# jibanCat/gp_dla_detection

Measured on AMD Instinct MI355X. Metric: sample log-likelihoods/sec (n~1500,k=20), higher is better.
Workload: dtype f64; 1 GPU; BASELINE configs[1]: synthetic spectra, fused Voigt + low-rank log-evidence sweep, HBM-resident; spectra_per_gpu=1000, pixels=1500, k=20, dla_samples=10000, num_lines=3, parallelism=spectra sharded over 1 GPU(s), RCCL all-gather of the 15-column posterior table

## Files before the change

gp_dla_detection_amd/csrc/sweep_kernels.hpp:

```cpp
#pragma once
#include <hip/hip_runtime.h>
#include <stdint.h>

#include <type_traits>
#include <utility>

#include "faddeeva.hpp"
#include "near_tables.hpp"

namespace gpdla {

typedef double d4 __attribute__((ext_vector_type(4)));

typedef float f4 __attribute__((ext_vector_type(4)));

template <typename T> struct Mat;
template <> struct Mat<double> {
  using acc_t = d4;
  static __device__ __forceinline__ acc_t mfma(double a, double b, acc_t c) {
    return __builtin_amdgcn_mfma_f64_16x16x4f64(a, b, c, 0, 0, 0);
  }
  static __device__ __forceinline__ int sample_of(int jj, int r) { return jj + 4 * r; }
  static __device__ __forceinline__ int jj_of(int sample) { return sample & 3; }
  static __device__ __forceinline__ int reg_of(int sample) { return sample >> 2; }
// ... 427 lines not shown
  p = fma(p, r, 0.16666666666666666);
  p = fma(p, r, 0.5);
  p = fma(p, r, 1.0);
  p = fma(p, r, 1.0);
  return ldexp(p, (int)n);
}

constexpr double kE1 = 0x1.7fffffffd940ep+0, kE2 = 0x1.e0000294b4cbcp+1, kE3 = 0x1.a3f92a26b3728p+3,
                 kE4 = 0x1.df9f0e43cd754p+5;
__device__ __forceinline__ double wing_lead(double rho, double e3v) {
  double t;
  asm("v_fma_f64 %0, %1, %2, %3" : "=v"(t) : "v"(rho), "s"(kE4), "v"(e3v));
  return t;
}

__device__ __forceinline__ double wing_core(double x2, double y2) {
  const double rho = fast_rcp(x2 + y2);
  double t = fma(kE4, rho, kE3);
  t = fma(t, rho, kE2);
  t = fma(t, rho, kE1);
  t = fma(t, rho, 1.0);
  t = fma(-2.0 * y2 * rho, rho, t);
  return rho * t;
}

__device__ __forceinline__ void glds16(const double *gsrc, double *lds_wave_base) {
  const uint32_t lds = __builtin_amdgcn_readfirstlane(
      (uint32_t)(uintptr_t)(__attribute__((address_space(3))) void *)lds_wave_base);
  asm volatile("s_mov_b32 m0, %1\n\ts_nop 0\n\tglobal_load_lds_dwordx4 %0, off"
               :
               : "v"(gsrc), "s"(lds)
               : "memory", "m0");
}
__device__ __forceinline__ void glds_wait() {
  __builtin_amdgcn_s_waitcnt(0x0F70);
  asm volatile("" ::: "memory");
}

constexpr int kRecordPoolPad = 8;
__device__ __forceinline__ void glds_quad(const double *gsrc, uint32_t lds, int count) {
  if (count >= 4)
    asm volatile("s_mov_b32 m0, %1\n\ts_nop 0\n\tglobal_load_lds_dwordx4 %0, off\n\t"
                 "global_load_lds_dwordx4 %0, off offset:1024\n\tglobal_load_lds_dwordx4 %0, off offset:2048\n\t"
                 "global_load_lds_dwordx4 %0, off offset:3072"
                 :
                 : "v"(gsrc), "s"(lds)
                 : "memory", "m0");
  else if (count == 3)
    asm volatile("s_mov_b32 m0, %1\n\ts_nop 0\n\tglobal_load_lds_dwordx4 %0, off\n\t"
                 "global_load_lds_dwordx4 %0, off offset:1024\n\tglobal_load_lds_dwordx4 %0, off offset:2048"
                 :
                 : "v"(gsrc), "s"(lds)
                 : "memory", "m0");
  else if (count == 2)
    asm volatile("s_mov_b32 m0, %1\n\ts_nop 0\n\tglobal_load_lds_dwordx4 %0, off\n\t"
                 "global_load_lds_dwordx4 %0, off offset:1024"
                 :
                 : "v"(gsrc), "s"(lds)
                 : "memory", "m0");
  else if (count == 1)
    asm volatile("s_mov_b32 m0, %1\n\ts_nop 0\n\tglobal_load_lds_dwordx4 %0, off" : : "v"(gsrc), "s"(lds) : "memory", "m0");
}
template <int KIB, int WAVES>
__device__ __forceinline__ void glds_chunk(const double *src, uint32_t lds, int wave, int lane) {
  constexpr int PER = (KIB + WAVES - 1) / WAVES;
  const int first = wave * PER;
// ... 414 lines not shown
  return q_s + ld_s + e[0];
#else
  if (role != 0) return NAN;
  if (TW <= 14)
    return factor_rows<ES::ROWS, ES::LPS, 20>(e + half * ncols, s & (ES::LPS - 1), k, voff, q_s, ld_s, n_kept);
#ifndef GPDLA_EXP_LDSEPI
  if constexpr (TW > 30 && ES::LPS == 16) {
    Rows16<40> R;
    load_rows16<40>(R, e, s, k, voff);
    return factor_rows16<40>(R, k, q_s, ld_s, n_kept);
  }
#endif
  return factor_lds<ES::ROWS, ES::LPS>(e + half * ncols, s & (ES::LPS - 1), k, voff, q_s, ld_s, n_kept);
#endif
}

__device__ __forceinline__ double near_poly(const double *line_tab, double ax) {
  const bool core = ax < 8.0;
  const double u = core ? ax * 8.0 : (ax - 8.0) * 2.0;
  const int i = (int)u;
  const double t = (u - (double)i) - 0.5;
  const double *c = line_tab + (size_t)((core ? 0 : kNearCore) + i) * kNearCoef;
  double cf[kNearCoef];
#pragma unroll
  for (int k = 0; k < kNearCoef; ++k) cf[k] = c[k];
  double p = cf[kNearCoef - 1];
#pragma unroll
  for (int k = kNearCoef - 2; k >= 0; --k) p = fma(p, t, cf[k]);
  return p;
}

__device__ __forceinline__ uint32_t hi_word(double v) { return (uint32_t)__double2hiint(v); }

__device__ __forceinline__ double wing_sum3(double lamP, double msa, double msb, double msc, double cs,
                                            bool *near) {
  const double xa = fma(lamP, msa, -cs), xb = fma(lamP, msb, -cs), xc = fma(lamP, msc, -cs);
  const double sa = fma(xa, xa, g_lines.y2[0]), sb = fma(xb, xb, g_lines.y2[1]), sc = fma(xc, xc, g_lines.y2[2]);
  static_assert(__builtin_bit_cast(unsigned long long, 900.0) == 0x408C200000000000ull, "bits of 900.0");
  *near = min(min(hi_word(sa), hi_word(sb)), hi_word(sc)) < 0x408C2000u;
  const double pab = sa * sb, pbc = sb * sc, pac = sa * sc;
  const double rinv = fast_rcp(pab * sc);
  const double ra = rinv * pbc, rb = rinv * pac, rc = rinv * pab;
  double ta = ra * kE4 + kE3, tb = rb * kE4 + kE3, tc = rc * kE4 + kE3;
  ta = fma(ta, ra, g_lines.t2[0]); tb = fma(tb, rb, g_lines.t2[1]); tc = fma(tc, rc, g_lines.t2[2]);
  ta = fma(ta, ra, kE1); tb = fma(tb, rb, kE1); tc = fma(tc, rc, kE1);
  ta = fma(ta, ra, 1.0); tb = fma(tb, rb, 1.0); tc = fma(tc, rc, 1.0);
  return fma(g_lines.cwing[2], rc * tc, fma(g_lines.cwing[1], rb * tb, g_lines.cwing[0] * (ra * ta)));
}

__device__ __forceinline__ double wing_sum3_rcp4(double lamP, double msa, double msb, double msc, double cs,
                                                 bool *near, double d, double *inv_d) {
  const double xa = fma(lamP, msa, -cs), xb = fma(lamP, msb, -cs), xc = fma(lamP, msc, -cs);
  const double sa = fma(xa, xa, g_lines.y2[0]), sb = fma(xb, xb, g_lines.y2[1]), sc = fma(xc, xc, g_lines.y2[2]);
  *near = min(min(hi_word(sa), hi_word(sb)), hi_word(sc)) < 0x408C2000u;
  const double pab = sa * sb, pabc = pab * sc;
  const double rinv = fast_rcp(pabc * d);
  *inv_d = rinv * pabc;
  const double r3 = rinv * d;
  const double rc = r3 * pab, r2 = r3 * sc;
  const double ra = r2 * sb, rb = r2 * sa;
  const double e3v = kE3;
  double ta = wing_lead(ra, e3v), tb = wing_lead(rb, e3v), tc = wing_lead(rc, e3v);
  ta = fma(ta, ra, g_lines.t2[0]); tb = fma(tb, rb, g_lines.t2[1]); tc = fma(tc, rc, g_lines.t2[2]);
  ta = fma(ta, ra, kE1); tb = fma(tb, rb, kE1); tc = fma(tc, rc, kE1);
  ta = fma(ta, ra, 1.0); tb = fma(tb, rb, 1.0); tc = fma(tc, rc, 1.0);
  return fma(g_lines.cwing[2], rc * tc, fma(g_lines.cwing[1], rb * tb, g_lines.cwing[0] * (ra * ta)));
}

constexpr int kRing2 = 33;
constexpr int kExpTab = 64;

struct ExpState {
  double r, tabv;
  int ni;
};
__device__ __forceinline__ ExpState exp_table_begin(double x, const double *tab) {
  ExpState e;
  const double nf = rint(x * 92.33248261689366);
  asm("v_cvt_i32_f64 %0, %1" : "=v"(e.ni) : "v"(nf));
  e.tabv = tab[e.ni & (kExpTab - 1)];
  e.r = fma(-nf, 0.010830424667801708, x);
  e.r = fma(-nf, 2.8447437476627285e-11, e.r);
  return e;
}
__device__ __forceinline__ double exp_table_end(const ExpState &e) {
  double p, c4 = 0.041666666666666664, c3 = 0.16666666666666666;
  asm("v_fma_f64 %0, %1, %2, %3" : "=v"(p) : "s"(0.008333333333333333), "v"(e.r), "v"(c4));
  asm("v_fma_f64 %0, %1, %2, %3" : "=v"(p) : "v"(p), "v"(e.r), "v"(c3));
  p = fma(p, e.r, 0.5);
  p = fma(p, e.r, 1.0);
  p = fma(p, e.r, 1.0);
  return ldexp(e.tabv * p, e.ni >> 6);
}
constexpr double kExpScale = 92.33248261689366;
__device__ __forceinline__ ExpState exp_table_begin_scaled(double t, const double *tab) {
  ExpState e;
  const double nf = rint(t);
  asm("v_cvt_i32_f64 %0, %1" : "=v"(e.ni) : "v"(nf));
  e.tabv = tab[e.ni & (kExpTab - 1)];
// ... 15 lines not shown
__device__ __forceinline__ double exp_table(double x, const double *tab) {
  return exp_table_end(exp_table_begin(x, tab));
}
__device__ __forceinline__ double exp_table_scaled(double t, const double *tab) {
  return exp_table_end_scaled(exp_table_begin_scaled(t, tab));
}

template <int LINES>
__device__ __forceinline__ double total_near(double lamP, double m0, double m1, double m2,
                                             const double *mult_lds, int L) {
  const double c_light = g_lines.c, inv_s = g_lines.inv_sqrt2_sigma;
  const double *tab = g_lines.near_poly;
  double total = 0.0;
  if (LINES > 0) {
    const double mm[3] = {m0, m1, m2};
#pragma unroll
    for (int j = 0; j < (LINES > 0 ? LINES : 1); ++j) {
      const double ax = fabs((lamP * mm[j < 3 ? j : 0] - c_light) * inv_s);
      const double f = ax < 30.0
                           ? 1.7724538509055159 * g_lines.leading[j] * near_poly(tab + j * kNearLineDoubles, ax)
                           : g_lines.cwing[j] * wing_core(ax * ax, g_lines.y2[j]);
      total += f;
    }
  } else {
    for (int j = 0; j < L; ++j) {
      const double ax = fabs((lamP * mult_lds[j] - c_light) * inv_s);
      const double f = ax < 30.0
                           ? 1.7724538509055159 * g_lines.leading[j] * near_poly(tab + j * kNearLineDoubles, ax)
                           : g_lines.cwing[j] * wing_core(ax * ax, g_lines.y2[j]);
      total += f;
    }
  }
  return total;
}

constexpr int kLineUnroll = 4;
__device__ __forceinline__ double wing_sum_runtime(double rho, double cs, int L, bool *near_out) {
  double total = 0.0;
  bool near = false;
  int j0 = 0;
  for (; j0 + kLineUnroll <= L; j0 += kLineUnroll) {
    double f[kLineUnroll];
#pragma unroll
    for (int u = 0; u < kLineUnroll; ++u) {
      const double x = fma(rho, g_lines.wing[j0 + u].kms, -cs);
      const double x2 = x * x;
      near |= x2 < 900.0;
      f[u] = wing_core(x2, g_lines.wing[j0 + u].y2);
    }
#pragma unroll
    for (int u = 0; u < kLineUnroll; ++u) total = fma(g_lines.wing[j0 + u].cwing, f[u], total);
  }
  for (; j0 < L; ++j0) {
    const double x = fma(rho, g_lines.wing[j0].kms, -cs);
    const double x2 = x * x;
    near |= x2 < 900.0;
    total = fma(g_lines.wing[j0].cwing, wing_core(x2, g_lines.wing[j0].y2), total);
  }
  *near_out = near;
  return total;
}

__device__ __forceinline__ double total_near_at(double lamP, double one_plus_z, int L) {
  const double c_light = g_lines.c, inv_s = g_lines.inv_sqrt2_sigma;
  const double *tab = g_lines.near_poly;
  double total = 0.0;
// ... 70 lines not shown
  if (tid < kExpTab) exp_tab[tid] = exp2((double)tid * (1.0 / kExpTab));
  double *my_ring = ring + (size_t)(wave * kSamplesPerWave + s) * kRing2 + jj;
  const double *lam = a.lam_pad + m.lam_off;
  const int n_pad = m.n_u + 6;
  const double nscale64 = -nhi * g_lines.inv_sqrt2pi_sigma * kInvSqrtPi * kExpScale;
  const double *rec_base = a.records + m.rec_off * (int64_t)RD;
  const int nchunks = (m.steps + kChunkSteps - 1) / kChunkSteps;

  static_assert((kChunkSteps * RD) % 128 == 0, "a chunk is a whole number of KiB");
  const int wave_s = __builtin_amdgcn_readfirstlane(wave);
  const uint32_t stage_lds = __builtin_amdgcn_readfirstlane(lds_address(stage));
  auto issue_chunk = [&](int c) {
    glds_chunk<kChunkSteps * RD / 128, WAVES>(rec_base + (size_t)c * kChunkSteps * RD,
                                              stage_lds + (uint32_t)(c & 1) * (uint32_t)(kChunkSteps * RD * 8), wave_s, lane);
  };
  issue_chunk(0);

  const double c_light = g_lines.c, inv_s = g_lines.inv_sqrt2_sigma;
  double ms_r[LINES > 0 ? LINES : 1];
#pragma unroll
  for (int j = 0; j < (LINES > 0 ? LINES : 0); ++j) ms_r[j] = mult_r[j] * inv_s;
  const double cs = c_light * inv_s;
#define GPDLA_TOTAL_ACCURATE(lamP)                                                        \
  total_near<LINES>((lamP), mult_r[0], mult_r[LINES > 1 ? 1 : 0], mult_r[LINES > 2 ? 2 : 0], \
                    my_mult, L)
#define GPDLA_RAW_ACCURATE(lamP) exp_table_scaled(nscale64 * GPDLA_TOTAL_ACCURATE(lamP), exp_tab)

  __syncthreads();
  for (int c3 = 0; c3 < 3; ++c3) {
    const double lam0 = lam[min(4 * c3 + jj, n_pad - 1)];
    double v;
    if (LINES == 3) {
      bool near0;
      v = exp_table_scaled(nscale64 * wing_sum3(lam0, ms_r[0], ms_r[LINES > 1 ? 1 : 0], ms_r[LINES > 2 ? 2 : 0],
                                                cs, &near0), exp_tab);
      if (__any(near0)) v = GPDLA_RAW_ACCURATE(lam0);
    } else {
      v = GPDLA_RAW_ACCURATE(lam0);
    }
    my_ring[4 * c3] = v;
    my_ring[4 * c3 + 16] = v;
  }

  acc_t acc[NTW];
#pragma unroll
  for (int c = 0; c < NTW; ++c) acc[c] = acc_t{0, 0, 0, 0};
  double quad_sum = 0.0, dprod = 1.0;
  double xw[kXW] = {0.0, 0.0}, xu[kXU] = {0.0, 0.0, 0.0, 0.0};
  int dexp = 0;
  const int tile0 = role * NTW;
  [[maybe_unused]] const int nw = TS == 1 ? TW : max(0, min(NTW, TW - tile0));
  const double tap0 = g_lines.taps[0], tap1 = g_lines.taps[1], tap2 = g_lines.taps[2],
               tap3 = g_lines.taps[3];

  glds_wait();
  __syncthreads();

#ifdef GPDLA_STAMP
  uint32_t st_sum[8] = {0, 0, 0, 0, 0, 0, 0, 0}, st_prev;
  {
    unsigned long long t0_;
    asm volatile("s_memtime %0\n\ts_waitcnt lgkmcnt(0)" : "=s"(t0_)::"memory");
    st_prev = (uint32_t)t0_;
  }
#endif
  for (int c0 = 0; c0 < nchunks; c0 += UN) {
#pragma unroll
  for (int hc = 0; hc < UN; ++hc) {
    const int c = c0 + hc;
// ... 1 lines not shown
    __builtin_amdgcn_s_waitcnt(0x0F70);
    GPDLA_ST(4)
    if (c + 1 < nchunks) issue_chunk(c + 1);
    GPDLA_ST(5)
    const double *buf = stage + (size_t)(UN > 1 ? hc : (c & 1)) * kChunkSteps * RD;
    double lam_next = 0.0;
#pragma unroll
    for (int tt = 0; tt < kChunkSteps; ++tt) {
      const int rn = c * kChunkSteps + tt;
      if (rn < m.steps) {
        const double *rec = buf + (size_t)tt * RD;
        const double *extra = rec + NT * TD;
        const int slot_p = kChunkSteps >= 4 ? (4 * tt) & 15 : (kChunkSteps == 2 ? 4 * (2 * hc + tt) : ((4 * rn) & 15));
        const int slot_w = (slot_p + 12) & 15;
        if (tt > 0) __builtin_amdgcn_s_waitcnt(0xC07F);
        const double *mine = extra + extras_row(NT, 1) * jj;
        const double lamP = tt == 0 ? extra[extras_lam_stride(NT) * jj + extras_lam(NT, 0)] : lam_next;
        const double *g = my_ring + slot_p;
        const double g0 = g[0], g1 = g[1], g2 = g[2], g3 = g[3], g4 = g[4], g5 = g[5], g6 = g[6];
        const double2 p01 = *reinterpret_cast<const double2 *>(mine);
        const double2 p23 = *reinterpret_cast<const double2 *>(mine + 2);
        const double py = p01.x, pmu = p01.y, pom = p23.x, pnu = p23.y;
        __builtin_amdgcn_sched_barrier(0);
        double absorb = g3 * tap3;
        absorb = fma(g0 + g6, tap0, absorb);
        absorb = fma(g1 + g5, tap1, absorb);
        absorb = fma(g2 + g4, tap2, absorb);
        if (is_null) absorb = 1.0;
        const double a2 = absorb * absorb;
        const double d = fma(pom, a2, pnu);
        double inv_d;
        double total;
        bool near;
        if (LINES == 3) {
          total = wing_sum3_rcp4(lamP, ms_r[0], ms_r[LINES > 1 ? 1 : 0], ms_r[LINES > 2 ? 2 : 0], cs, &near, d, &inv_d);
        } else {
          inv_d = fast_rcp(d);
          total = 0.0;
          near = false;
          for (int j = 0; j < L; ++j) {
            const double x = fma(lamP, my_mult[j] * inv_s, -cs);
            const double x2 = x * x;
            near |= x2 < 900.0;
            total = fma(g_lines.cwing[j], wing_core(x2, g_lines.y2[j]), total);
          }
        }
        GPDLA_ST(0)
#ifndef GPDLA_ABLATE_NOSLOW
        if (__builtin_expect(__any(near), 0)) total = GPDLA_TOTAL_ACCURATE(lamP);
#endif
        GPDLA_ST(1)
        const ExpState es = exp_table_begin_scaled(nscale64 * total, exp_tab);
        __builtin_amdgcn_sched_barrier(0);
        const T *bt = reinterpret_cast<const T *>(rec) + (size_t)tile0 * 64 + lane;
        T bop[NTW];
#ifdef GPDLA_ABLATE_NOBFRAG
#pragma unroll
        for (int cc = 0; cc < NTW; ++cc) bop[cc] = (T)(lane + cc) * (T)lamP;
        (void)bt;
#else
#pragma unroll
        for (int cc = 0; cc < NTW; ++cc) bop[cc] = bt[(size_t)cc * 64];
#endif
        __builtin_amdgcn_sched_barrier(0);
        double raw = exp_table_end_scaled(es);
#ifdef GPDLA_ABLATE_NOVOIGT
        raw = lamP * 1e-4;
#endif
        my_ring[slot_w] = raw;
        my_ring[slot_w + 16] = raw;
        const double r = fma(-absorb, pmu, py);
        const double w = a2 * inv_d;
        const double ri = r * inv_d;
        const double u = absorb * ri;
        quad_sum = fma(r, ri, quad_sum);
        dprod *= d;
        if (kChunkSteps == 1 || (tt & 1)) {
          dexp += __builtin_amdgcn_frexp_exp(dprod);
          dprod = __builtin_amdgcn_frexp_mant(dprod);
        }
        if (tt + 1 < kChunkSteps) {
          lam_next = extra[RD + extras_lam_stride(NT) * jj + extras_lam(NT, 0)];
// ... 282 lines not shown
```

gp_dla_detection_amd/csrc/sweep_slim_body.hpp:

```cpp
template <int LINES>
__global__ __launch_bounds__(kSlimWaves * 64, 2) void GPDLA_SWEEP_SLIM_KERNEL(GPDLA_SWEEP_SLIM_ARGS a) {
  static_assert(LINES == 3 || LINES == 0, "three lines at compile time, or a run-time count");
  extern __shared__ double smem[];
  constexpr int WAVES = kSlimWaves, CH = kSlimSweepCH;
  const int64_t xj = blockIdx.x >> 3;
  const int64_t pos = 8 * (xj / a.blocks_per_quasar) + (blockIdx.x & 7);
  const int bq = (int)(xj % a.blocks_per_quasar);
  if (pos >= a.nq) return;
  const int64_t q = a.order[pos];
  const QuasarMeta m = a.meta[q];
  if (m.status != 0) return;
  const int tid = threadIdx.x, wave = tid >> 6, lane = tid & 63;
  const int s = lane & 15, jj = lane >> 4;

  double *ring = smem;
  double *blocks = ring + kSlimSweepRingD;
  double *land = blocks + 2 * kSlimSweepBlock + wave * kSlimLand;
  const double *exp_pad = ring + 32;

  const int64_t slot0 = (int64_t)bq * (WAVES * kSamplesPerWave) + wave * kSamplesPerWave;
  const int64_t slot = slot0 + s;
  const bool is_sample = slot < a.S;
  const bool is_null = !is_sample;
  const int32_t sample = a.perm[is_sample ? slot : a.S - 1];
  const double z_dla = m.min_z_dla + (m.max_z_dla - m.min_z_dla) * a.offset_samples[sample];
  double nhi = a.nhi_samples[sample];
  if constexpr (std::is_same_v<GPDLA_SWEEP_SLIM_ARGS, BoxedSweepArgs> && LINES >= 0) {
    const double *box = sweep_box(a, q);
    nhi = exp10(box[2] + (box[3] - box[2]) * nhi);
  }
  [[maybe_unused]] double mult_r[3];
  [[maybe_unused]] const double opz = 1 + z_dla, inv_opz = 1.0 / opz;
  [[maybe_unused]] const int L = LINES > 0 ? LINES : a.num_lines;
  if constexpr (LINES == 3) {
#pragma unroll
    for (int j = 0; j < 3; ++j) mult_r[j] = g_lines.c / (g_lines.wavelength_cm[j] * (1 + z_dla)) / 1e8;
  }
  if (tid < kExpTab) ring[tid * kRing2 + 32] = exp2((double)tid * (1.0 / kExpTab));
  double *my_ring = ring + (size_t)(wave * kSamplesPerWave + s) * kRing2 + jj;
  const double *lam = a.lam_pad + m.lam_off;
  const int n_pad = m.n_u + 6;
  const double nscale64 = -nhi * g_lines.inv_sqrt2pi_sigma * kInvSqrtPi * kExpScale;
  const double *rec_base = a.records + m.rec_off * (int64_t)kSlimRec;
  const int nchunks = (m.steps + CH - 1) / CH;

  const int wave_s = __builtin_amdgcn_readfirstlane(wave);
  double *const raw_mine = blocks + kSlimSweepTileBuf + wave_s * kSlimRec;
  const double *const raw_src = rec_base + (size_t)wave_s * kSlimRec + 2 * lane;
  auto issue_chunk = [&](int c) {
    if (lane < kSlimRec / 2) glds16(raw_src + (size_t)c * CH * kSlimRec, raw_mine + (c & 1) * kSlimSweepBlock);
  };
  const double *land_src = rec_base + (size_t)wave_s * kSlimRec;
  const int src_rows = 4 * kSlimExtras + 16 * jj + 2 * (s & 7);
  const int src_x = kSlimExtras * (lane >> 1) + 4 + 2 * (lane & 1);
  auto issue_private = [&](int c) {
    const double *rec = land_src + (size_t)c * CH * kSlimRec;
    glds16(rec + src_rows, land);
    if (lane < 8) glds16(rec + src_x, land + 4 * 32);
  };
  const double *row = land + 32 * jj + s;
  const double *bc = land + 4 * 32 + 4 * jj;
  const double *a8 = s < 8 ? row : bc + (slim_pair_i(8, s) - 16);
  const double *b8 = s < 8 ? row + 8 : bc + (slim_pair_j(8, s) - 16);
  struct Operands {
    double mc, o[5], p8;
  };
  auto expand_load = [&](int t0, int t1, Operands &x) {
    x.mc = row[0];
#pragma unroll
    for (int t = t0; t < t1; ++t) {
      if (t == 8) {
        x.o[t - t0] = a8[0];
        x.p8 = b8[0];
      } else {
        x.o[t - t0] = t == 0 ? x.mc : t < 8 ? row[t] : bc[t - 9];
      }
    }
  };
  auto expand_store = [&](double *dst, int t0, int t1, const Operands &x) {
#pragma unroll
    for (int t = t0; t < t1; ++t) dst[t * 64] = (t == 8 ? x.p8 : x.mc) * x.o[t - t0];
  };
  double *const xd0 = blocks + (size_t)wave_s * kSlimStepTiles + lane;
  const double *const tb0 = blocks + lane;
  const double *const mb0 = blocks + kSlimSweepTileBuf + kSlimExtras * jj;
  const double *const ub0 = blocks + kSlimSweepTileBuf + 4 * kSlimExtras + lane;
  auto pinned = [](const double *p) {
    uint32_t v = lds_address(p);
    asm volatile("" : "+v"(v));
    return (double *)(__attribute__((address_space(3))) double *)(uintptr_t)v;
  };

  issue_private(0);
  issue_chunk(0);

  const double c_light = g_lines.c, inv_s = g_lines.inv_sqrt2_sigma;
  [[maybe_unused]] double ms_r[3];
  if constexpr (LINES == 3) {
#pragma unroll
    for (int j = 0; j < 3; ++j) ms_r[j] = mult_r[j] * inv_s;
  }
  const double cs = c_light * inv_s;
  auto optical_sum = [&](double lamP) -> double {
    if constexpr (LINES == 3) {
      bool near;
      double total = wing_sum3(lamP, ms_r[0], ms_r[1], ms_r[2], cs, &near);
      if (__builtin_expect(__any(near), 0)) total = total_near<3>(lamP, mult_r[0], mult_r[1], mult_r[2], nullptr, 3);
      return total;
    } else {
      bool near;
      double total = wing_sum_runtime(lamP * inv_opz, cs, L, &near);
      if (__builtin_expect(__any(near), 0)) total = total_near_at(lamP, opz, L);
      return total;
    }
  };

  __syncthreads();
  for (int c3 = 0; c3 < 3; ++c3) {
    const double lam0 = lam[min(4 * c3 + jj, n_pad - 1)];
    const double tot = optical_sum(lam0);
    const ExpState es0 = exp_ring_begin_scaled(nscale64 * tot, exp_pad);
    const double v = exp_table_end_scaled(es0);
    my_ring[4 * c3] = v;
    my_ring[4 * c3 + 16] = v;
  }

  d4 acc[14];
#pragma unroll
  for (int c = 0; c < 14; ++c) acc[c] = d4{0, 0, 0, 0};
  double quad_sum = 0.0, dprod = 1.0;
  double xw[kXW] = {0.0, 0.0}, xu[kXU] = {0.0, 0.0, 0.0, 0.0};
  int dexp = 0;
  const double tap0 = g_lines.taps[0], tap1 = g_lines.taps[1], tap2 = g_lines.taps[2], tap3 = g_lines.taps[3];

  glds_wait();
  {
    const double mc = row[0];
    for (int t = 0; t < kSlimTilesW; ++t)
      xd0[t * 64] = (t == 8 ? b8[0] : mc) * (t == 8 ? a8[0] : t == 0 ? mc : t < 8 ? row[t] : bc[t - 9]);
  }
  __builtin_amdgcn_s_waitcnt(0xC07F);
  if (nchunks > 1) issue_private(1);
  glds_wait();
  __syncthreads();

  double n0 = my_ring[0], n1 = my_ring[1], n2 = my_ring[2], n3 = my_ring[3], n4 = my_ring[4], n5 = my_ring[5], n6 = my_ring[6];
  for (int c = 0; c < nchunks; ++c) {
    __builtin_amdgcn_s_waitcnt(0x0070);
    if (c + 1 < nchunks) issue_chunk(c + 1);
    const int par = (c & 1) * kSlimSweepBlock;
    const double *tbuf = pinned(tb0 + par);
    const double *mine0 = pinned(mb0 + par);
    const double *ubuf = pinned(ub0 + par);
    double *xdst = pinned(xd0 + (kSlimSweepBlock - par));
    double lam_next = 0.0;
    double2 n01 = {0.0, 0.0}, n23 = {0.0, 0.0};
#pragma unroll
    for (int tt = 0; tt < CH; ++tt) {
      const int rn = c * CH + tt;
      constexpr int kXS = 3;
      constexpr int kT0[3] = {0, 5, 9}, kT1[3] = {5, 9, 13};
      if (tt == kXS && c + 2 < nchunks) issue_private(c + 2);
      if (rn < m.steps) {
        const double *tl = tbuf + (size_t)tt * kSlimStepTiles;
        const double *mine = mine0 + (size_t)tt * kSlimRec;
        const int slot_p = (4 * tt) & 15;
        const int slot_w = (slot_p + 12) & 15;
        if (tt > 0) __builtin_amdgcn_s_waitcnt(0xC07F);
        const double lamP = tt == 0 ? mine[10] : lam_next;
        double g0 = n0, g1 = n1, g2 = n2, g3 = n3, g4 = n4, g5 = n5, g6 = n6;
        double2 p01 = n01, p23 = n23;
        if (tt == 0) {
          p01 = *reinterpret_cast<const double2 *>(mine);
          p23 = *reinterpret_cast<const double2 *>(mine + 2);
        }
        const double py = p01.x, pmu = p01.y, pom = p23.x, pnu = p23.y;
        __builtin_amdgcn_sched_barrier(0);
        [[maybe_unused]] WingFront wf;
        [[maybe_unused]] bool near = false;
        if constexpr (LINES == 3) {
          if (tt == 0) {
            wf = wing3_front(lamP, ms_r[0], ms_r[1], ms_r[2], cs, &near);
            __builtin_amdgcn_sched_barrier(0);
          }
        }
        double absorb = g3 * tap3;
        absorb = fma(g0 + g6, tap0, absorb);
        absorb = fma(g1 + g5, tap1, absorb);
        absorb = fma(g2 + g4, tap2, absorb);
        if (is_null) absorb = 1.0;
        const double a2 = absorb * absorb;
        const double d = fma(pom, a2, pnu);
        double inv_d;
        double total;
        if constexpr (LINES == 3) {
          if (tt > 0) wf = wing3_front(lamP, ms_r[0], ms_r[1], ms_r[2], cs, &near);
          total = wing3_back_rcp4(wf, d, &inv_d);
#ifndef SLIM_EXP_NONEAR
          if (__builtin_expect(__any(near), 0)) total = total_near<3>(lamP, mult_r[0], mult_r[1], mult_r[2], nullptr, 3);
#endif
        } else {
          total = optical_sum(lamP);
          inv_d = fast_rcp(d);
        }
        const ExpState es = exp_ring_begin_scaled(nscale64 * total, exp_pad);
        __builtin_amdgcn_sched_barrier(0);
        double bop[14];
#pragma unroll
        for (int cc = 0; cc < kSlimTilesW; ++cc) bop[cc] = tl[cc * 64];
        bop[13] = ubuf[(size_t)tt * kSlimRec];
        __builtin_amdgcn_sched_barrier(0);
        const double pser = exp_series_scaled(es);
        const double r = fma(-absorb, pmu, py);
        const double w = a2 * inv_d;
        const double ri = r * inv_d;
        const double u = absorb * ri;
        quad_sum = fma(r, ri, quad_sum);
        dprod *= d;
        if (tt & 1) {
          dexp += __builtin_amdgcn_frexp_exp(dprod);
          dprod = __builtin_amdgcn_frexp_mant(dprod);
        }
        __builtin_amdgcn_sched_barrier(0);
        const double raw = exp_finish_scaled(es, pser);
        my_ring[slot_w] = raw;
        my_ring[slot_w + 16] = raw;
        Operands x;
        if (tt < kXS) expand_load(kT0[tt < kXS ? tt : 0], kT1[tt < kXS ? tt : 0], x);
        if (tt + 1 < CH) lam_next = mine[kSlimRec + 10];
        __builtin_amdgcn_sched_barrier(0);
        constexpr int kSplit = 11;
        const double2 xp = *reinterpret_cast<const double2 *>(mine + 8);
// ... 66 lines not shown
```

gp_dla_detection_amd/csrc/sweep_slim_kernel.hpp:

```cpp
#pragma once
#include <type_traits>

#include "sweep_kernels.hpp"

namespace gpdla {

constexpr int kSlimExtras = 12;
constexpr int kSlimRec = 4 * kSlimExtras + 64;
constexpr int kSlimCH = 8;
constexpr int kSlimTilesW = 13;
constexpr int kSlimStepTiles = kSlimTilesW * 64;
constexpr int kSlimTileBuf = kSlimCH * kSlimStepTiles;
constexpr int kSlimRawBuf = kSlimCH * kSlimRec;
constexpr int kSlimLand = 4 * 32 + 4 * 4;
constexpr int kSlimBlock = kSlimTileBuf + kSlimRawBuf;
static_assert((kSlimBlock * 8) % 512 == 0, "both parities reachable with ds_read2st64 offsets");
static_assert((kSlimCH * kSlimRec) % 128 == 0, "a raw chunk is a whole number of KiB");
constexpr int kSlimWaves = 4;
constexpr int kSlimSweepCH = 4;
constexpr int kSlimSweepRingD = kSlimWaves * kSamplesPerWave * kRing2;
constexpr int kSlimSweepTileBuf = kSlimSweepCH * kSlimStepTiles;
constexpr int kSlimSweepBlock = kSlimSweepTileBuf + kSlimSweepCH * kSlimRec;
constexpr int kSlimLdsDoubles = kSlimSweepRingD + 2 * kSlimSweepBlock + kSlimWaves * kSlimLand;
static_assert(kSlimSweepCH == kSlimWaves, "wave w expands, and copies, K-step w of the next chunk");
// ... 70 lines not shown
__device__ __forceinline__ ExpState exp_ring_begin_scaled(double t, const double *ring_pad) {
  ExpState e;
  const double nf = rint(t);
  asm("v_cvt_i32_f64 %0, %1" : "=v"(e.ni) : "v"(nf));
  e.tabv = ring_pad[(e.ni & (kExpTab - 1)) * kRing2];
  e.r = t - nf;
  return e;
}

__device__ __forceinline__ double exp_series_scaled(const ExpState &e) {
  constexpr double L = 0.010830424696249145;
  constexpr double c1 = L, c2 = L * L / 2, c3 = L * L * L / 6, c4 = L * L * L * L / 24, c5 = L * L * L * L * L / 120;
  double p;
  const double c4v = c4;
  asm("v_fma_f64 %0, %1, %2, %3" : "=v"(p) : "s"(c5), "v"(e.r), "v"(c4v));
  asm("v_fma_f64 %0, %1, %2, %3" : "=v"(p) : "v"(p), "v"(e.r), "s"(c3));
  asm("v_fma_f64 %0, %1, %2, %3" : "=v"(p) : "v"(p), "v"(e.r), "s"(c2));
  asm("v_fma_f64 %0, %1, %2, %3" : "=v"(p) : "v"(p), "v"(e.r), "s"(c1));
  return fma(p, e.r, 1.0);
}
__device__ __forceinline__ double exp_finish_scaled(const ExpState &e, double p) { return ldexp(e.tabv * p, e.ni >> 6); }

struct WingFront {
  double sa, sb, sc, pab, pabc;
};
__device__ __forceinline__ WingFront wing3_front(double lamP, double msa, double msb, double msc, double cs, bool *near) {
  WingFront f;
  const double xa = fma(lamP, msa, -cs), xb = fma(lamP, msb, -cs), xc = fma(lamP, msc, -cs);
  f.sa = fma(xa, xa, g_lines.y2[0]), f.sb = fma(xb, xb, g_lines.y2[1]), f.sc = fma(xc, xc, g_lines.y2[2]);
  *near = min(min(hi_word(f.sa), hi_word(f.sb)), hi_word(f.sc)) < 0x408C2000u;
  f.pab = f.sa * f.sb, f.pabc = f.pab * f.sc;
  return f;
}
__device__ __forceinline__ double wing3_back_rcp4(const WingFront &f, double d, double *inv_d) {
  const double rinv = fast_rcp(f.pabc * d);
  *inv_d = rinv * f.pabc;
  const double r3 = rinv * d;
  const double rc = r3 * f.pab, r2 = r3 * f.sc;
  const double ra = r2 * f.sb, rb = r2 * f.sa;
  const double e3v = kE3;
  double ta = wing_lead(ra, e3v), tb = wing_lead(rb, e3v), tc = wing_lead(rc, e3v);
  ta = fma(ta, ra, g_lines.t2[0]); tb = fma(tb, rb, g_lines.t2[1]); tc = fma(tc, rc, g_lines.t2[2]);
  ta = fma(ta, ra, kE1); tb = fma(tb, rb, kE1); tc = fma(tc, rc, kE1);
  ta = fma(ta, ra, 1.0); tb = fma(tb, rb, 1.0); tc = fma(tc, rc, 1.0);
  return fma(g_lines.cwing[2], rc * tc, fma(g_lines.cwing[1], rb * tb, g_lines.cwing[0] * (ra * ta)));
}

__device__ __forceinline__ double slim_factor_pass(const d4 (&acc)[14], const double (&xw)[kXW],
                                                   const double (&xu)[kXU], int p, double *Eg, int lane, int k,
                                                   double quad_sum, double logd_sum, int n_kept,
                                                   int *sigma_out, bool *writer) {
  using ES = EpilogueShape<13, 1>;
  constexpr int voff = (13 + 1) * 16;
  constexpr int ncols = ES::stride(16);
  const int s = lane & 15, jj = lane >> 4;
  const int half = s >> 3;
  const int sigma = Mat<double>::sample_of(jj, ES::RPP * p + half);
  const double q_s = __shfl(quad_sum, sigma + 16 * jj);
  const double ld_s = __shfl(logd_sum, sigma + 16 * jj);
  double *e = Eg + (size_t)(jj * ES::RPP) * ncols;
#pragma unroll
  for (int cc = 0; cc < 14; ++cc) {
    const int at = cc < kSlimTilesW ? slim_pos(cc, s) : voff + s;
#pragma unroll
    for (int h = 0; h < ES::RPP; ++h) e[h * ncols + at] = acc[cc][ES::RPP * p + h];
  }
  {
    const int r = Mat<double>::reg_of(s);
    if (jj == 0 && r / ES::RPP == p) {
      double *es = Eg + (size_t)(Mat<double>::jj_of(s) * ES::RPP + r % ES::RPP) * ncols;
#pragma unroll
      for (int x = 0; x < kXW; ++x) es[kXWColumn + x] = xw[x];
#pragma unroll
      for (int x = 0; x < kXU; ++x) es[voff + kXUColumn + x] = xu[x];
    }
  }
  __builtin_amdgcn_fence(__ATOMIC_RELEASE, "wavefront");
  __builtin_amdgcn_wave_barrier();
// ... 18 lines not shown
```

gp_dla_detection_amd/csrc/sweep_split_kernel.hpp:

```cpp
#pragma once
#include "sweep_kernels.hpp"

namespace gpdla {

constexpr int kSplitRing = 65;

__host__ __device__ constexpr size_t sweep_split_lds_doubles(int num_lines_runtime) {
  constexpr int RD = 56 * 64 + record_extras(56);
  return kExpTab + 2 * 2 * (size_t)RD
         + 2 * 16 * kSplitRing
         + 2 * 2 * 2 * 4 * 64
         + 2 * 4 * 2 * 16
         + (size_t)2 * 16 * num_lines_runtime;
}

template <int LINES>
__global__ __launch_bounds__(512) void k_sweep_split(SweepArgs a) {
  extern __shared__ double smem[];
  constexpr int WAVES = 8, TS = 4, NTW = 14, NT = 56, TW = 52, CH = 2;
  constexpr int RD = NT * 64 + record_extras(NT);
  const int64_t xj = blockIdx.x >> 3;
  const int64_t pos = 8 * (xj / a.blocks_per_quasar) + (blockIdx.x & 7);
  const int bq = (int)(xj % a.blocks_per_quasar);
  if (pos >= a.nq) return;
// ... 25 lines not shown
#pragma unroll
    for (int j = 0; j < LINES; ++j) mult_r[j] = g_lines.c / (g_lines.wavelength_cm[j] * (1 + z_dla)) / 1e8;
  } else if (role == 0 && jj == 0) {
    for (int j = 0; j < L; ++j) my_mult[j] = g_lines.c / (g_lines.wavelength_cm[j] * (1 + z_dla)) / 1e8;
  }
  if (tid < kExpTab) exp_tab[tid] = exp2((double)tid * (1.0 / kExpTab));
  const double *lam = a.lam_pad + m.lam_off;
  const PixelRow *pix = a.pix + m.pix_off;
  const int n_pad = m.n_u + 6;
  const double nscale64 = -nhi * g_lines.inv_sqrt2pi_sigma * kInvSqrtPi * kExpScale;
  const double *rec_base = a.records + m.rec_off * (int64_t)RD;
  const int nchunks = (m.steps + CH - 1) / CH;
  const int niter = (m.steps + 3) / 4;
  const double c_light = g_lines.c, inv_s = g_lines.inv_sqrt2_sigma;
  double ms_r[LINES > 0 ? LINES : 1];
#pragma unroll
  for (int j = 0; j < (LINES > 0 ? LINES : 0); ++j) ms_r[j] = mult_r[j] * inv_s;
  const double cs = c_light * inv_s;
  const double tap0 = g_lines.taps[0], tap1 = g_lines.taps[1], tap2 = g_lines.taps[2], tap3 = g_lines.taps[3];

  static_assert((CH * RD) % 128 == 0, "a chunk is a whole number of KiB");
  const int wave_s = __builtin_amdgcn_readfirstlane(wave);
  const uint32_t stage_lds = __builtin_amdgcn_readfirstlane(lds_address(stage));
  auto issue_chunk = [&](int c) {
    glds_chunk<CH * RD / 128, WAVES>(rec_base + (size_t)c * CH * RD, stage_lds + (uint32_t)(c & 1) * (uint32_t)(CH * RD * 8),
                                     wave_s, lane);
  };
  issue_chunk(0);

  double *my_ring = ring + (size_t)(group * 16 + s) * kSplitRing;
  auto raw_of = [&](double lamP) -> double {
    double total;
    bool near;
    if (LINES == 3) {
      total = wing_sum3(lamP, ms_r[0], ms_r[LINES > 1 ? 1 : 0], ms_r[LINES > 2 ? 2 : 0], cs, &near);
    } else {
      total = 0.0;
      near = false;
      for (int j = 0; j < L; ++j) {
        const double x = fma(lamP, my_mult[j] * inv_s, -cs);
        const double x2 = x * x;
        near |= x2 < 900.0;
        total = fma(g_lines.cwing[j], wing_core(x2, g_lines.y2[j]), total);
      }
    }
    if (__builtin_expect(__any(near), 0))
      total = total_near<LINES>(lamP, mult_r[0], mult_r[LINES > 1 ? 1 : 0], mult_r[LINES > 2 ? 2 : 0], my_mult, L);
    return exp_table_scaled(nscale64 * total, exp_tab);
  };
  auto lam_of = [&](int tr) -> double { return lam[min(4 * tr + jj, n_pad - 1)]; };
  auto pix_of = [&](int t) -> PixelRow { return pix[4 * min(t, m.steps) + jj]; };

  double quad_sum = 0.0, dprod = 1.0;
  int dexp = 0;
  auto weights_of = [&](int t, const PixelRow &px, double *w_out, double *u_out) {
    const int p0 = 4 * t + jj;
    const double g0 = my_ring[p0 & 63], g1 = my_ring[(p0 + 1) & 63], g2 = my_ring[(p0 + 2) & 63],
                 g3 = my_ring[(p0 + 3) & 63], g4 = my_ring[(p0 + 4) & 63], g5 = my_ring[(p0 + 5) & 63],
                 g6 = my_ring[(p0 + 6) & 63];
    double absorb = fma(g6, tap0, g0 * tap0);
    double ab2 = fma(g5, tap1, g1 * tap1);
    absorb = fma(g2, tap2, absorb);
    ab2 = fma(g4, tap2, ab2);
    absorb = fma(g3, tap3, absorb) + ab2;
    if (is_null) absorb = 1.0;
    const double r = fma(-absorb, px.mu, px.y);
    const double a2 = absorb * absorb;
    const double d = fma(px.omega2, a2, px.nu);
    const double inv_d = fast_rcp(d);
    const double ri = r * inv_d;
    *w_out = a2 * inv_d;
    *u_out = absorb * ri;
    if (t < m.steps) {
      quad_sum = fma(r, ri, quad_sum);
      dprod *= d;
      dexp += __builtin_amdgcn_frexp_exp(dprod);
      dprod = __builtin_amdgcn_frexp_mant(dprod);
    }
  };
  auto wu_slot = [&](int par, int which, int step) -> double * {
// ... 128 lines not shown
```

gp_dla_detection_amd/csrc/sweep_split_slim_kernel.hpp:

```cpp
#pragma once
#include <type_traits>

#include "multi_kernels.hpp"
#include "sweep_split_kernel.hpp"

#ifndef S40_EPI_PW
#define S40_EPI_PW 4
#endif

namespace gpdla {
__host__ __device__ constexpr int vmcnt_imm(int n) { return (n & 15) | (7 << 4) | (15 << 8) | ((n >> 4) << 14); }
static_assert(vmcnt_imm(0) == 0x0F70, "the encoding glds_wait() uses");
}

namespace gpdla {

constexpr int kS40Row = 48;
constexpr int kS40Rec = 4 * kS40Row;
constexpr int kS40CH = 8;
constexpr int kS40Zero = 40, kS40One = 46;
constexpr int kS40Ring = 129;
constexpr int kS40Tiles = 56, kS40TilesW = 52, kS40NTW = 7;
constexpr int kS40Lead = 20;
static_assert(kS40CH <= kRecordPoolPad, "a chunk copy may run this far past a quasar's last record");
// ... 163 lines not shown
    for (int j = 0; j < (LINES > 0 ? LINES : 0); ++j) ms_r[j] = mult_r[j] * inv_s;
    cs = g_lines.c * inv_s;
    my_ring = ring + (size_t)(group * 16 + s) * kS40Ring;
  }
  const double tap0 = g_lines.taps[0], tap1 = g_lines.taps[1], tap2 = g_lines.taps[2], tap3 = g_lines.taps[3];

  static_assert((CH * kS40Rec) % 128 == 0, "a chunk is a whole number of KiB");
  const uint32_t stage_lds = __builtin_amdgcn_readfirstlane(lds_address(stage));
  auto issue_chunk = [&](int c) {
    glds_chunk<CH * kS40Rec / 128, 8>(rec_base + (size_t)c * CH * kS40Rec,
                                      stage_lds + (uint32_t)(c & 1) * (uint32_t)(CH * kS40Rec * 8), wave_s, lane);
  };
  issue_chunk(0);

  uint32_t pa[NTW], pb[NTW];
#pragma unroll
  for (int cc = 0; cc < NTW; ++cc) {
    const int T = wave_s * NTW + cc;
    pa[cc] = stage_lds + (uint32_t)(jj * kS40Row + s40_a(T, s)) * 8u;
    pb[cc] = stage_lds + (uint32_t)(jj * kS40Row + s40_b(T, s)) * 8u;
    asm volatile("" : "+v"(pa[cc]), "+v"(pb[cc]));
  }
  auto lds_at = [](uint32_t addr, int byte_off) -> double {
    return ((const __attribute__((address_space(3))) double *)(uintptr_t)addr)[byte_off / 8];
  };
  auto wu_at = [&](int par, int g, int which, int step) -> double * {
    return wu + ((((size_t)par * 2 + g) * 2 + which) * CH + step) * 64 + lane;
  };
  const int tail_which = wave_s == 7 ? 1 : 0;

  auto raw_of = [&](double lamP) -> double {
    double total;
    bool near;
    if (LINES == 3) {
      total = wing_sum3(lamP, ms_r[0], ms_r[LINES > 1 ? 1 : 0], ms_r[LINES > 2 ? 2 : 0], cs, &near);
    } else {
      total = wing_sum_runtime(lamP * inv_opz, cs, L, &near);
    }
    if (__builtin_expect(__any(near), 0)) {
      if constexpr (LINES > 0) total = total_near<LINES>(lamP, mult_r[0], mult_r[LINES > 1 ? 1 : 0], mult_r[LINES > 2 ? 2 : 0], nullptr, L);
      else total = total_near_at(lamP, opz, L);
    }
    return exp_table_scaled(nscale64 * total, exp_tab);
  };
  auto lam_of = [&](int tr) -> double { return lam[min(4 * tr + jj, n_pad - 1)]; };
  auto pix_of = [&](int t) -> PixelRow { return pix[4 * min(t, m.steps) + jj]; };
  const int p_last = 4 * m.steps + jj;
  auto gather = [&](int t, double (&r)[NDR]) {
    const int p = min(4 * t + jj, p_last);
#pragma unroll
    for (int j = 0; j < NDR; ++j) r[j] = rows[j][p];
  };

  double quad_sum = 0.0, dprod = 1.0;
  int dexp = 0;
  auto weigh = [&](int t, const PixelRow &px, double absorb, double *w_out, double *u_out) {
    if (is_null) absorb = 1.0;
    const double r = fma(-absorb, px.mu, px.y);
    const double a2 = absorb * absorb;
    const double d = fma(px.omega2, a2, px.nu);
    const double inv_d = fast_rcp(d);
    *w_out = a2 * inv_d;
    if constexpr (kMulti) {
      *u_out = absorb * r * inv_d;
      if (t < m.steps) quad_sum = fma(r * r, inv_d, quad_sum);
    } else {
      const double ri = r * inv_d;
      *u_out = absorb * ri;
      if (t < m.steps) quad_sum = fma(r, ri, quad_sum);
    }
    if (t < m.steps) {
      dprod *= d;
      dexp += __builtin_amdgcn_frexp_exp(dprod);
// ... 271 lines not shown
```

Baseline: 70.96 million evals/s.

## Reuse wing terms in near-line fallback and use scalar-base LDS loads

When any lane is near a line center, the slow path no longer recomputes all three lines. It reuses the wing terms the fast path already computed and evaluates the near polynomial only for lines whose squared distance is below threshold in some lane. The slim sweep also switches the global-to-LDS copies to a uniform scalar base pointer plus per-lane VGPR offsets, and pins several LDS base pointers, to cut per-lane address arithmetic. The near-line path now clamps ax just below 30 and picks per-line formulas, which could change numerics slightly near the boundary.

```diff
diff --git a/gp_dla_detection_amd/csrc/sweep_kernels.hpp b/gp_dla_detection_amd/csrc/sweep_kernels.hpp
--- a/gp_dla_detection_amd/csrc/sweep_kernels.hpp
+++ b/gp_dla_detection_amd/csrc/sweep_kernels.hpp
@@ -483,6 +483,19 @@
                : "v"(gsrc), "s"(lds)
                : "memory", "m0");
 }
+__device__ __forceinline__ const double *uniform_pointer(const double *p) {
+  const uint64_t v = (uint64_t)(uintptr_t)p;
+  const uint32_t lo = __builtin_amdgcn_readfirstlane((uint32_t)v), hi = __builtin_amdgcn_readfirstlane((uint32_t)(v >> 32));
+  return (const double *)(uintptr_t)(((uint64_t)hi << 32) | lo);
+}
+__device__ __forceinline__ void glds16_at(const double *sbase, uint32_t lane_bytes, double *lds_wave_base) {
+  const uint32_t lds = __builtin_amdgcn_readfirstlane(
+      (uint32_t)(uintptr_t)(__attribute__((address_space(3))) void *)lds_wave_base);
+  asm volatile("s_mov_b32 m0, %2\n\ts_nop 0\n\tglobal_load_lds_dwordx4 %0, %1"
+               :
+               : "v"(lane_bytes), "s"(sbase), "s"(lds)
+               : "memory", "m0");
+}
 __device__ __forceinline__ void glds_wait() {
   __builtin_amdgcn_s_waitcnt(0x0F70);
   asm volatile("" ::: "memory");
@@ -963,8 +976,12 @@
 
 __device__ __forceinline__ uint32_t hi_word(double v) { return (uint32_t)__double2hiint(v); }
 
+struct WingLines3 {
+  double s[3], q[3];
+};
+
 __device__ __forceinline__ double wing_sum3(double lamP, double msa, double msb, double msc, double cs,
-                                            bool *near) {
+                                            bool *near, WingLines3 *lines = nullptr) {
   const double xa = fma(lamP, msa, -cs), xb = fma(lamP, msb, -cs), xc = fma(lamP, msc, -cs);
   const double sa = fma(xa, xa, g_lines.y2[0]), sb = fma(xb, xb, g_lines.y2[1]), sc = fma(xc, xc, g_lines.y2[2]);
   static_assert(__builtin_bit_cast(unsigned long long, 900.0) == 0x408C200000000000ull, "bits of 900.0");
@@ -976,11 +993,13 @@
   ta = fma(ta, ra, g_lines.t2[0]); tb = fma(tb, rb, g_lines.t2[1]); tc = fma(tc, rc, g_lines.t2[2]);
   ta = fma(ta, ra, kE1); tb = fma(tb, rb, kE1); tc = fma(tc, rc, kE1);
   ta = fma(ta, ra, 1.0); tb = fma(tb, rb, 1.0); tc = fma(tc, rc, 1.0);
-  return fma(g_lines.cwing[2], rc * tc, fma(g_lines.cwing[1], rb * tb, g_lines.cwing[0] * (ra * ta)));
+  const double qa = ra * ta, qb = rb * tb, qc = rc * tc;
+  if (lines) *lines = WingLines3{{sa, sb, sc}, {qa, qb, qc}};
+  return fma(g_lines.cwing[2], qc, fma(g_lines.cwing[1], qb, g_lines.cwing[0] * qa));
 }
 
 __device__ __forceinline__ double wing_sum3_rcp4(double lamP, double msa, double msb, double msc, double cs,
-                                                 bool *near, double d, double *inv_d) {
+                                                 bool *near, double d, double *inv_d, WingLines3 *lines) {
   const double xa = fma(lamP, msa, -cs), xb = fma(lamP, msb, -cs), xc = fma(lamP, msc, -cs);
   const double sa = fma(xa, xa, g_lines.y2[0]), sb = fma(xb, xb, g_lines.y2[1]), sc = fma(xc, xc, g_lines.y2[2]);
   *near = min(min(hi_word(sa), hi_word(sb)), hi_word(sc)) < 0x408C2000u;
@@ -995,7 +1014,9 @@
   ta = fma(ta, ra, g_lines.t2[0]); tb = fma(tb, rb, g_lines.t2[1]); tc = fma(tc, rc, g_lines.t2[2]);
   ta = fma(ta, ra, kE1); tb = fma(tb, rb, kE1); tc = fma(tc, rc, kE1);
   ta = fma(ta, ra, 1.0); tb = fma(tb, rb, 1.0); tc = fma(tc, rc, 1.0);
-  return fma(g_lines.cwing[2], rc * tc, fma(g_lines.cwing[1], rb * tb, g_lines.cwing[0] * (ra * ta)));
+  const double qa = ra * ta, qb = rb * tb, qc = rc * tc;
+  *lines = WingLines3{{sa, sb, sc}, {qa, qb, qc}};
+  return fma(g_lines.cwing[2], qc, fma(g_lines.cwing[1], qb, g_lines.cwing[0] * qa));
 }
 
 constexpr int kRing2 = 33;
@@ -1077,6 +1098,26 @@
     }
   }
   return total;
+}
+
+__device__ __forceinline__ double near_lines3(double lamP, double m0, double m1, double m2, const WingLines3 &w) {
+  const double c_light = g_lines.c, inv_s = g_lines.inv_sqrt2_sigma;
+  const double mm[3] = {m0, m1, m2};
+  double coef[3], term[3];
+#pragma unroll
+  for (int j = 0; j < 3; ++j) {
+    coef[j] = g_lines.cwing[j];
+    term[j] = w.q[j];
+    const bool near_j = hi_word(w.s[j]) < 0x408C2000u;
+    if (__any(near_j)) {
+      if (near_j) {
+        const double ax = fmin(fabs((lamP * mm[j] - c_light) * inv_s), 0x1.fffffffffffffp+4);
+        coef[j] = 1.7724538509055159 * g_lines.leading[j];
+        term[j] = near_poly(g_lines.near_poly + j * kNearLineDoubles, ax);
+      }
+    }
+  }
+  return fma(coef[2], term[2], fma(coef[1], term[1], coef[0] * term[0]));
 }
 
 constexpr int kLineUnroll = 4;
@@ -1213,9 +1254,10 @@
     double v;
     if (LINES == 3) {
       bool near0;
-      v = exp_table_scaled(nscale64 * wing_sum3(lam0, ms_r[0], ms_r[LINES > 1 ? 1 : 0], ms_r[LINES > 2 ? 2 : 0],
-                                                cs, &near0), exp_tab);
-      if (__any(near0)) v = GPDLA_RAW_ACCURATE(lam0);
+      WingLines3 wl;
+      double total = wing_sum3(lam0, ms_r[0], ms_r[LINES > 1 ? 1 : 0], ms_r[LINES > 2 ? 2 : 0], cs, &near0, &wl);
+      if (__any(near0)) total = near_lines3(lam0, mult_r[0], mult_r[LINES > 1 ? 1 : 0], mult_r[LINES > 2 ? 2 : 0], wl);
+      v = exp_table_scaled(nscale64 * total, exp_tab);
     } else {
       v = GPDLA_RAW_ACCURATE(lam0);
     }
@@ -1283,8 +1325,9 @@
         double inv_d;
         double total;
         bool near;
+        [[maybe_unused]] WingLines3 wl;
         if (LINES == 3) {
-          total = wing_sum3_rcp4(lamP, ms_r[0], ms_r[LINES > 1 ? 1 : 0], ms_r[LINES > 2 ? 2 : 0], cs, &near, d, &inv_d);
+          total = wing_sum3_rcp4(lamP, ms_r[0], ms_r[LINES > 1 ? 1 : 0], ms_r[LINES > 2 ? 2 : 0], cs, &near, d, &inv_d, &wl);
         } else {
           inv_d = fast_rcp(d);
           total = 0.0;
@@ -1298,7 +1341,10 @@
         }
         GPDLA_ST(0)
 #ifndef GPDLA_ABLATE_NOSLOW
-        if (__builtin_expect(__any(near), 0)) total = GPDLA_TOTAL_ACCURATE(lamP);
+        if (__builtin_expect(__any(near), 0)) {
+          if (LINES == 3) total = near_lines3(lamP, mult_r[0], mult_r[LINES > 1 ? 1 : 0], mult_r[LINES > 2 ? 2 : 0], wl);
+          else total = GPDLA_TOTAL_ACCURATE(lamP);
+        }
 #endif
         GPDLA_ST(1)
         const ExpState es = exp_table_begin_scaled(nscale64 * total, exp_tab);
diff --git a/gp_dla_detection_amd/csrc/sweep_slim_body.hpp b/gp_dla_detection_amd/csrc/sweep_slim_body.hpp
--- a/gp_dla_detection_amd/csrc/sweep_slim_body.hpp
+++ b/gp_dla_detection_amd/csrc/sweep_slim_body.hpp
@@ -46,17 +46,18 @@
 
   const int wave_s = __builtin_amdgcn_readfirstlane(wave);
   double *const raw_mine = blocks + kSlimSweepTileBuf + wave_s * kSlimRec;
-  const double *const raw_src = rec_base + (size_t)wave_s * kSlimRec + 2 * lane;
-  auto issue_chunk = [&](int c) {
-    if (lane < kSlimRec / 2) glds16(raw_src + (size_t)c * CH * kSlimRec, raw_mine + (c & 1) * kSlimSweepBlock);
-  };
-  const double *land_src = rec_base + (size_t)wave_s * kSlimRec;
-  const int src_rows = 4 * kSlimExtras + 16 * jj + 2 * (s & 7);
-  const int src_x = kSlimExtras * (lane >> 1) + 4 + 2 * (lane & 1);
-  auto issue_private = [&](int c) {
-    const double *rec = land_src + (size_t)c * CH * kSlimRec;
-    glds16(rec + src_rows, land);
-    if (lane < 8) glds16(rec + src_x, land + 4 * 32);
+  const double *const my_rec0 = uniform_pointer(rec_base + (size_t)wave_s * kSlimRec);
+  constexpr size_t kChunkDoubles = (size_t)CH * kSlimRec;
+  uint32_t off_raw = 16u * (uint32_t)lane;
+  auto issue_chunk = [&](int c, const double *my_rec) {
+    if (lane < kSlimRec / 2) glds16_at(my_rec, off_raw, raw_mine + (c & 1) * kSlimSweepBlock);
+  };
+  uint32_t off_rows = 8u * (uint32_t)(4 * kSlimExtras + 16 * jj + 2 * (s & 7));
+  uint32_t off_x = 8u * (uint32_t)(kSlimExtras * (lane >> 1) + 4 + 2 * (lane & 1));
+  asm volatile("" : "+v"(off_raw), "+v"(off_rows), "+v"(off_x));
+  auto issue_private = [&](const double *my_rec) {
+    glds16_at(my_rec, off_rows, land);
+    if (lane < 8) glds16_at(my_rec, off_x, land + 4 * 32);
   };
   const double *row = land + 32 * jj + s;
   const double *bc = land + 4 * 32 + 4 * jj;
@@ -81,18 +82,19 @@
 #pragma unroll
     for (int t = t0; t < t1; ++t) dst[t * 64] = (t == 8 ? x.p8 : x.mc) * x.o[t - t0];
   };
-  double *const xd0 = blocks + (size_t)wave_s * kSlimStepTiles + lane;
-  const double *const tb0 = blocks + lane;
-  const double *const mb0 = blocks + kSlimSweepTileBuf + kSlimExtras * jj;
-  const double *const ub0 = blocks + kSlimSweepTileBuf + 4 * kSlimExtras + lane;
   auto pinned = [](const double *p) {
     uint32_t v = lds_address(p);
     asm volatile("" : "+v"(v));
     return (double *)(__attribute__((address_space(3))) double *)(uintptr_t)v;
   };
-
-  issue_private(0);
-  issue_chunk(0);
+  double *const xd1 = pinned(blocks + kSlimSweepBlock + (size_t)wave_s * kSlimStepTiles + lane);
+  double *const xd0 = xd1 - kSlimSweepBlock;
+  const double *const tb0 = pinned(blocks + lane);
+  const double *const mb0 = pinned(blocks + kSlimSweepTileBuf + kSlimExtras * jj);
+  const double *const ub0 = pinned(blocks + kSlimSweepTileBuf + 4 * kSlimExtras + lane);
+
+  issue_private(my_rec0);
+  issue_chunk(0, my_rec0);
 
   const double c_light = g_lines.c, inv_s = g_lines.inv_sqrt2_sigma;
   [[maybe_unused]] double ms_r[3];
@@ -104,8 +106,9 @@
   auto optical_sum = [&](double lamP) -> double {
     if constexpr (LINES == 3) {
       bool near;
-      double total = wing_sum3(lamP, ms_r[0], ms_r[1], ms_r[2], cs, &near);
-      if (__builtin_expect(__any(near), 0)) total = total_near<3>(lamP, mult_r[0], mult_r[1], mult_r[2], nullptr, 3);
+      WingLines3 wl;
+      double total = wing_sum3(lamP, ms_r[0], ms_r[1], ms_r[2], cs, &near, &wl);
+      if (__builtin_expect(__any(near), 0)) total = near_lines3(lamP, mult_r[0], mult_r[1], mult_r[2], wl);
       return total;
     } else {
       bool near;
@@ -140,19 +143,20 @@
       xd0[t * 64] = (t == 8 ? b8[0] : mc) * (t == 8 ? a8[0] : t == 0 ? mc : t < 8 ? row[t] : bc[t - 9]);
   }
   __builtin_amdgcn_s_waitcnt(0xC07F);
-  if (nchunks > 1) issue_private(1);
+  if (nchunks > 1) issue_private(my_rec0 + kChunkDoubles);
   glds_wait();
   __syncthreads();
 
   double n0 = my_ring[0], n1 = my_ring[1], n2 = my_ring[2], n3 = my_ring[3], n4 = my_ring[4], n5 = my_ring[5], n6 = my_ring[6];
-  for (int c = 0; c < nchunks; ++c) {
+  const double *next_rec = my_rec0 + kChunkDoubles;
+  for (int c = 0; c < nchunks; ++c, next_rec += kChunkDoubles) {
     __builtin_amdgcn_s_waitcnt(0x0070);
-    if (c + 1 < nchunks) issue_chunk(c + 1);
+    if (c + 1 < nchunks) issue_chunk(c + 1, next_rec);
     const int par = (c & 1) * kSlimSweepBlock;
     const double *tbuf = pinned(tb0 + par);
     const double *mine0 = pinned(mb0 + par);
     const double *ubuf = pinned(ub0 + par);
-    double *xdst = pinned(xd0 + (kSlimSweepBlock - par));
+    double *xdst = pinned(xd1 - par);
     double lam_next = 0.0;
     double2 n01 = {0.0, 0.0}, n23 = {0.0, 0.0};
 #pragma unroll
@@ -160,7 +164,7 @@
       const int rn = c * CH + tt;
       constexpr int kXS = 3;
       constexpr int kT0[3] = {0, 5, 9}, kT1[3] = {5, 9, 13};
-      if (tt == kXS && c + 2 < nchunks) issue_private(c + 2);
+      if (tt == kXS && c + 2 < nchunks) issue_private(next_rec + kChunkDoubles);
       if (rn < m.steps) {
         const double *tl = tbuf + (size_t)tt * kSlimStepTiles;
         const double *mine = mine0 + (size_t)tt * kSlimRec;
@@ -195,9 +199,10 @@
         double total;
         if constexpr (LINES == 3) {
           if (tt > 0) wf = wing3_front(lamP, ms_r[0], ms_r[1], ms_r[2], cs, &near);
-          total = wing3_back_rcp4(wf, d, &inv_d);
+          WingLines3 wl;
+          total = wing3_back_rcp4(wf, d, &inv_d, &wl);
 #ifndef SLIM_EXP_NONEAR
-          if (__builtin_expect(__any(near), 0)) total = total_near<3>(lamP, mult_r[0], mult_r[1], mult_r[2], nullptr, 3);
+          if (__builtin_expect(__any(near), 0)) total = near_lines3(lamP, mult_r[0], mult_r[1], mult_r[2], wl);
 #endif
         } else {
           total = optical_sum(lamP);
diff --git a/gp_dla_detection_amd/csrc/sweep_slim_kernel.hpp b/gp_dla_detection_amd/csrc/sweep_slim_kernel.hpp
--- a/gp_dla_detection_amd/csrc/sweep_slim_kernel.hpp
+++ b/gp_dla_detection_amd/csrc/sweep_slim_kernel.hpp
@@ -126,7 +126,7 @@
   f.pab = f.sa * f.sb, f.pabc = f.pab * f.sc;
   return f;
 }
-__device__ __forceinline__ double wing3_back_rcp4(const WingFront &f, double d, double *inv_d) {
+__device__ __forceinline__ double wing3_back_rcp4(const WingFront &f, double d, double *inv_d, WingLines3 *lines) {
   const double rinv = fast_rcp(f.pabc * d);
   *inv_d = rinv * f.pabc;
   const double r3 = rinv * d;
@@ -137,7 +137,9 @@
   ta = fma(ta, ra, g_lines.t2[0]); tb = fma(tb, rb, g_lines.t2[1]); tc = fma(tc, rc, g_lines.t2[2]);
   ta = fma(ta, ra, kE1); tb = fma(tb, rb, kE1); tc = fma(tc, rc, kE1);
   ta = fma(ta, ra, 1.0); tb = fma(tb, rb, 1.0); tc = fma(tc, rc, 1.0);
-  return fma(g_lines.cwing[2], rc * tc, fma(g_lines.cwing[1], rb * tb, g_lines.cwing[0] * (ra * ta)));
+  const double qa = ra * ta, qb = rb * tb, qc = rc * tc;
+  *lines = WingLines3{{f.sa, f.sb, f.sc}, {qa, qb, qc}};
+  return fma(g_lines.cwing[2], qc, fma(g_lines.cwing[1], qb, g_lines.cwing[0] * qa));
 }
 
 __device__ __forceinline__ double slim_factor_pass(const d4 (&acc)[14], const double (&xw)[kXW],
diff --git a/gp_dla_detection_amd/csrc/sweep_split_kernel.hpp b/gp_dla_detection_amd/csrc/sweep_split_kernel.hpp
--- a/gp_dla_detection_amd/csrc/sweep_split_kernel.hpp
+++ b/gp_dla_detection_amd/csrc/sweep_split_kernel.hpp
@@ -81,8 +81,9 @@
   auto raw_of = [&](double lamP) -> double {
     double total;
     bool near;
+    [[maybe_unused]] WingLines3 wl;
     if (LINES == 3) {
-      total = wing_sum3(lamP, ms_r[0], ms_r[LINES > 1 ? 1 : 0], ms_r[LINES > 2 ? 2 : 0], cs, &near);
+      total = wing_sum3(lamP, ms_r[0], ms_r[LINES > 1 ? 1 : 0], ms_r[LINES > 2 ? 2 : 0], cs, &near, &wl);
     } else {
       total = 0.0;
       near = false;
@@ -93,8 +94,10 @@
         total = fma(g_lines.cwing[j], wing_core(x2, g_lines.y2[j]), total);
       }
     }
-    if (__builtin_expect(__any(near), 0))
-      total = total_near<LINES>(lamP, mult_r[0], mult_r[LINES > 1 ? 1 : 0], mult_r[LINES > 2 ? 2 : 0], my_mult, L);
+    if (__builtin_expect(__any(near), 0)) {
+      if (LINES == 3) total = near_lines3(lamP, mult_r[0], mult_r[LINES > 1 ? 1 : 0], mult_r[LINES > 2 ? 2 : 0], wl);
+      else total = total_near<LINES>(lamP, mult_r[0], mult_r[LINES > 1 ? 1 : 0], mult_r[LINES > 2 ? 2 : 0], my_mult, L);
+    }
     return exp_table_scaled(nscale64 * total, exp_tab);
   };
   auto lam_of = [&](int tr) -> double { return lam[min(4 * tr + jj, n_pad - 1)]; };
diff --git a/gp_dla_detection_amd/csrc/sweep_split_slim_kernel.hpp b/gp_dla_detection_amd/csrc/sweep_split_slim_kernel.hpp
--- a/gp_dla_detection_amd/csrc/sweep_split_slim_kernel.hpp
+++ b/gp_dla_detection_amd/csrc/sweep_split_slim_kernel.hpp
@@ -219,13 +219,15 @@
   auto raw_of = [&](double lamP) -> double {
     double total;
     bool near;
+    [[maybe_unused]] WingLines3 wl;
     if (LINES == 3) {
-      total = wing_sum3(lamP, ms_r[0], ms_r[LINES > 1 ? 1 : 0], ms_r[LINES > 2 ? 2 : 0], cs, &near);
+      total = wing_sum3(lamP, ms_r[0], ms_r[LINES > 1 ? 1 : 0], ms_r[LINES > 2 ? 2 : 0], cs, &near, &wl);
     } else {
       total = wing_sum_runtime(lamP * inv_opz, cs, L, &near);
     }
     if (__builtin_expect(__any(near), 0)) {
-      if constexpr (LINES > 0) total = total_near<LINES>(lamP, mult_r[0], mult_r[LINES > 1 ? 1 : 0], mult_r[LINES > 2 ? 2 : 0], nullptr, L);
+      if constexpr (LINES == 3) total = near_lines3(lamP, mult_r[0], mult_r[1], mult_r[2], wl);
+      else if constexpr (LINES > 0) total = total_near<LINES>(lamP, mult_r[0], mult_r[LINES > 1 ? 1 : 0], mult_r[LINES > 2 ? 2 : 0], nullptr, L);
       else total = total_near_at(lamP, opz, L);
     }
     return exp_table_scaled(nscale64 * total, exp_tab);
```

Result: faster. 71.94 million evals/s, median of 6 (+1.4%).
